# jgsimard/big-dreamer

Hardware: AMD Instinct MI355X
Metric: latent transitions/sec (RSSM + imagination) at batch=50 chunk=50 H=15 (higher is better)
Workload: dtype f32

## Files before the change

### big_dreamer_amd/csrc/bd_device.h

```cpp
#pragma once
#include <hip/hip_runtime.h>
#include <stdint.h>

namespace bd {

typedef float floatx4 __attribute__((ext_vector_type(4)));

#ifndef BD_WAVES
#define BD_WAVES 4
#endif
constexpr int kWaves = BD_WAVES;
constexpr int kThreads = kWaves * 64;
constexpr int kFragFloats = 256;

__device__ __forceinline__ floatx4 mfma16(float a, float b, floatx4 c) {
    return __builtin_amdgcn_mfma_f32_16x16x4f32(a, b, c, 0, 0, 0);
}

__host__ __device__ __forceinline__ int cdiv(int a, int b) { return (a + b - 1) / b; }

__device__ __forceinline__ int bd_tid() {
    int t = threadIdx.x;
    asm volatile("" : "+v"(t));
    return t;
// ... 210 lines not shown

#ifdef BD_STAMPS
#ifndef BD_STAMP_BLOCK
#define BD_STAMP_BLOCK 0
#endif
#ifndef BD_STAMP_THREAD
#define BD_STAMP_THREAD 0
#endif
static __device__ unsigned long long g_dstamps[64];
#define BD_DSTAMP(base, k)                                                                                  \
    do {                                                                                                    \
        if ((base) >= 0 && (base) + (k) < 64 && blockIdx.x == BD_STAMP_BLOCK && threadIdx.x == BD_STAMP_THREAD) \
            g_dstamps[(base) + (k)] = __builtin_amdgcn_s_memtime();                                          \
    } while (0)
#else
#define BD_DSTAMP(base, k)
#endif

__device__ __forceinline__ floatx4 tall_bias(const float* __restrict__ bias, int N, int nb, int lane) {
    const int col0 = nb * 16 + 4 * (lane >> 4);
    floatx4 b = floatx4{0.f, 0.f, 0.f, 0.f};
    if (bias != nullptr && col0 < N) {
        if (col0 + 4 <= N) {
            __builtin_memcpy(&b, bias + col0, 16);
        } else {
#pragma unroll
            for (int r = 0; r < 4; ++r)
                if (col0 + r < N) b[r] = bias[col0 + r];
        }
    }
    return b;
}

template <int NSEG, int RT, int NI, int D, bool TR = false>
__device__ __forceinline__ void linear_sweep(const Seg (&seg)[NSEG], int nb0, floatx4 (*acc)[RT]) {
    const int lane = bd_tid() & 63;
    constexpr bool kSplit = (NI * RT == 1);
    floatx4 acc2 = floatx4{0.f, 0.f, 0.f, 0.f};
#pragma unroll
    for (int s = 0; s < NSEG; ++s) {
        const int Kb = seg[s].Kb;
        const floatx4* __restrict__ X4 = reinterpret_cast<const floatx4*>(seg[s].X) + lane;
        const floatx4* __restrict__ W4 = reinterpret_cast<const floatx4*>(seg[s].W) + lane + (size_t)nb0 * Kb * 64;
        const size_t wstride = (size_t)kWaves * Kb * 64;
        pipelined_k<D>(
            Kb,
            [&](int kb) {
                LinFrag<RT, NI> f;
#pragma unroll
                for (int i = 0; i < NI; ++i) f.b[i] = W4[i * wstride + (size_t)kb * 64];
#pragma unroll
                for (int rt = 0; rt < RT; ++rt) f.a[rt] = X4[(rt * Kb + kb) * 64];
                return f;
            },
            [&](const LinFrag<RT, NI>& f) {
                if constexpr (kSplit) {
                    if constexpr (TR) {
                        acc[0][0] = mfma16(f.b[0][0], f.a[0][0], acc[0][0]);
                        acc2 = mfma16(f.b[0][1], f.a[0][1], acc2);
                        acc[0][0] = mfma16(f.b[0][2], f.a[0][2], acc[0][0]);
                        acc2 = mfma16(f.b[0][3], f.a[0][3], acc2);
                    } else {
                        acc[0][0] = mfma16(f.a[0][0], f.b[0][0], acc[0][0]);
                        acc2 = mfma16(f.a[0][1], f.b[0][1], acc2);
                        acc[0][0] = mfma16(f.a[0][2], f.b[0][2], acc[0][0]);
                        acc2 = mfma16(f.a[0][3], f.b[0][3], acc2);
                    }
                } else {
#pragma unroll
                    for (int j = 0; j < 4; ++j)
#pragma unroll
                        for (int i = 0; i < NI; ++i)
#pragma unroll
                            for (int rt = 0; rt < RT; ++rt)
                                acc[i][rt] = TR ? mfma16(f.b[i][j], f.a[rt][j], acc[i][rt]) : mfma16(f.a[rt][j], f.b[i][j], acc[i][rt]);
                }
            });
    }
    if constexpr (kSplit) acc[0][0] += acc2;
}

template <int NSEG, int RT, int NI, int D, bool TR = false, class Pre, class Epi>
__device__ __forceinline__ void linear_blocks(const Seg (&seg)[NSEG], const float* __restrict__ bias, int N, int nb0,
                                              Pre&& pre, Epi&& epi, int sb = -1) {
    const int lane = bd_tid() & 63;
    BD_DSTAMP(sb, 0);
    decltype(pre(0, 0)) pf[NI][RT];
#pragma unroll
    for (int i = 0; i < NI; ++i)
#pragma unroll
        for (int rt = 0; rt < RT; ++rt) pf[i][rt] = pre(rt, nb0 + i * kWaves);
    floatx4 acc[NI][RT];
#pragma unroll
    for (int i = 0; i < NI; ++i) {
        floatx4 b4;
        if constexpr (TR) {
            b4 = tall_bias(bias, N, nb0 + i * kWaves, lane);
        } else {
            const int col = (nb0 + i * kWaves) * 16 + (lane & 15);
            const float b = (bias != nullptr && col < N) ? bias[col] : 0.f;
            b4 = floatx4{b, b, b, b};
        }
#pragma unroll
        for (int rt = 0; rt < RT; ++rt) acc[i][rt] = b4;
    }
    BD_DSTAMP(sb, 1);
    linear_sweep<NSEG, RT, NI, D, TR>(seg, nb0, acc);
    BD_DSTAMP(sb, 2);
#pragma unroll
    for (int i = 0; i < NI; ++i)
#pragma unroll
        for (int rt = 0; rt < RT; ++rt) epi(rt, nb0 + i * kWaves, acc[i][rt], pf[i][rt]);
    BD_DSTAMP(sb, 3);
}

constexpr int kSplitPairs = 2;
constexpr int kHeadMaxN = 64;
constexpr int kHeadPlainFloats = 2 * 16 * kHeadMaxN;
constexpr int kSplitPartialFloats = kWaves * kSplitPairs * 2 * kFragFloats;
constexpr int kSplitScratchFloats = kSplitPartialFloats + kHeadPlainFloats;

template <int RT, int NSEG, bool TR = false, class Pre, class Epi>
__device__ __forceinline__ void tile_linear_splitk(const Seg (&seg)[NSEG], const float* __restrict__ bias, int N,
                                                   float* __restrict__ scratch, Pre&& pre, Epi&& epi) {
    const int lane = bd_tid() & 63, wave = bd_wave(bd_tid());
    const int Nb = (N + 15) >> 4;
    const int P = Nb * RT;
    const int my_nb = wave / RT, my_rt = wave - my_nb * RT;
    decltype(pre(0, 0)) pf{};
    floatx4 my_bias = floatx4{0.f, 0.f, 0.f, 0.f};
    if (wave < P) {
        pf = pre(my_rt, my_nb);
        if constexpr (TR) {
            my_bias = tall_bias(bias, N, my_nb, lane);
        } else {
            const int col = my_nb * 16 + (lane & 15);
            const float b = (bias != nullptr && col < N) ? bias[col] : 0.f;
            my_bias = floatx4{b, b, b, b};
        }
    }
// ... 16 lines not shown
                    if (kb < Kb && p < P) {
                        const int nb = p / RT, rt = p % RT;
                        xa[i][p] = X4[(rt * Kb + kb) * 64];
                        wb[i][p] = W4[((size_t)nb * Kb + kb) * 64];
                    }
                }
            }
#pragma unroll
            for (int i = 0; i < KW; ++i) {
                const int kb = kb0 + i * kWaves;
#pragma unroll
                for (int p = 0; p < kSplitPairs; ++p) {
                    if (kb < Kb && p < P) {
#pragma unroll
                        for (int j = 0; j < 4; ++j)
                            acc[p] = TR ? mfma16(wb[i][p][j], xa[i][p][j], acc[p]) : mfma16(xa[i][p][j], wb[i][p][j], acc[p]);
                    }
                }
            }
        }
    }
    floatx4* __restrict__ S4 = reinterpret_cast<floatx4*>(scratch);
#pragma unroll
    for (int p = 0; p < kSplitPairs; ++p)
        if (p < P) S4[(wave * kSplitPairs + p) * 64 + lane] = acc[p];
    lds_barrier();
    if (wave < P) {
        floatx4 r = my_bias;
        for (int w = 0; w < kWaves; ++w) r += S4[(w * kSplitPairs + wave) * 64 + lane];
        epi(my_rt, my_nb, r, pf);
    }
}

template <int RT, int NSEG, bool TR = false, class Pre, class Epi>
__device__ __forceinline__ void tile_linear_pre(const Seg (&seg)[NSEG], const float* __restrict__ bias, int N, Pre&& pre,
                                                Epi&& epi, float* __restrict__ scratch = nullptr, int sb = -1) {
    const int wave = bd_wave(bd_tid());
    const int Nb = (N + 15) >> 4;
    if (scratch != nullptr && Nb * RT <= kSplitPairs) {
        tile_linear_splitk<RT, NSEG, TR>(seg, bias, N, scratch, pre, epi);
        return;
    }
#ifndef BD_PIPE_D
#define BD_PIPE_D 2
#endif
    constexpr int D = BD_PIPE_D;
    for (int nb0 = wave; nb0 < Nb; nb0 += 2 * kWaves) {
        if (nb0 + kWaves < Nb) linear_blocks<NSEG, RT, 2, D, TR>(seg, bias, N, nb0, pre, epi, sb);
        else linear_blocks<NSEG, RT, 1, D, TR>(seg, bias, N, nb0, pre, epi, sb);
    }
}

template <int RT, int NSEG, class Epi>
__device__ __forceinline__ void tile_linear_g(const Seg (&seg)[NSEG], const float* __restrict__ bias, int N, Epi&& epi,
                                              float* __restrict__ scratch = nullptr, int sb = -1) {
    tile_linear_pre<RT, NSEG>(seg, bias, N, NoPre{}, [&](int rt, int nb, floatx4 acc, NoPreVal) { epi(rt, nb, acc); },
                              scratch, sb);
}

template <int RT, class Epi>
__device__ __forceinline__ void tile_linear(const float* __restrict__ X, int Kb, const float* __restrict__ Wp,
                                            const float* __restrict__ bias, int N, Epi&& epi,
                                            float* __restrict__ scratch = nullptr) {
    const Seg seg[1] = {{X, Wp, Kb}};
    tile_linear_g<RT, 1>(seg, bias, N, epi, scratch);
}

template <int NSEG, class Epi>
__device__ __forceinline__ void tile_linear_seg(const Seg (&seg)[NSEG], const float* __restrict__ bias, int N,
                                                Epi&& epi, float* __restrict__ scratch = nullptr, int sb = -1) {
    tile_linear_g<1, NSEG>(seg, bias, N, [&](int, int nb, floatx4 acc) { epi(nb, acc); }, scratch, sb);
}
template <int NSEG, class Epi>
__device__ __forceinline__ void tile_linear_seg_tr(const Seg (&seg)[NSEG], const float* __restrict__ bias, int N, Epi&& epi,
                                                   int sb = -1) {
    tile_linear_pre<1, NSEG, true>(seg, bias, N, NoPre{}, [&](int, int nb, floatx4 acc, NoPreVal) { epi(nb, acc); }, nullptr, sb);
}

constexpr int kTallMaxPer = 3;

template <int RT>
struct TallAcc {
    floatx4 main[kTallMaxPer][RT];
    floatx4 left;
};

__host__ __device__ __forceinline__ bool tall_shape_ok(int N, int RT) {
    const int Nb = (N + 15) >> 4, per = Nb / kWaves;
    return per <= kTallMaxPer && (Nb - per * kWaves) * RT <= kWaves;
}

__device__ __forceinline__ bool tall_left_pair(int Nb, int RT, int wave, int& rt, int& nb) {
    const int per = Nb / kWaves, nleft = (Nb - per * kWaves) * RT;
    if (wave >= nleft) return false;
    const int lb = wave / RT;
    rt = wave - lb * RT;
    nb = per * kWaves + lb;
    return true;
}

template <int RT, int NSEG>
__device__ __forceinline__ void tall_sweep(const Seg (&seg)[NSEG], const float* __restrict__ bias, int N, TallAcc<RT>& t) {
    const int lane = bd_tid() & 63, wave = bd_wave(bd_tid());
    const int Nb = (N + 15) >> 4, per = Nb / kWaves;
#pragma unroll
    for (int i = 0; i < kTallMaxPer; ++i) {
        const floatx4 b = i < per ? tall_bias(bias, N, wave + i * kWaves, lane) : floatx4{0.f, 0.f, 0.f, 0.f};
#pragma unroll
        for (int rt = 0; rt < RT; ++rt) t.main[i][rt] = b;
    }
    if (per == 3) linear_sweep<NSEG, RT, 3, 1, true>(seg, wave, t.main);
    else if (per == 2) linear_sweep<NSEG, RT, 2, 1, true>(seg, wave, t.main);
    else if (per == 1) linear_sweep<NSEG, RT, 1, 2, true>(seg, wave, t.main);
    int lrt = 0, lnb = 0;
    if (tall_left_pair(Nb, RT, wave, lrt, lnb)) {
        floatx4 one[1][1] = {{tall_bias(bias, N, lnb, lane)}};
        Seg s1[NSEG];
#pragma unroll
        for (int s = 0; s < NSEG; ++s) s1[s] = Seg{seg[s].X + (size_t)lrt * seg[s].Kb * kFragFloats, seg[s].W, seg[s].Kb};
        linear_sweep<NSEG, 1, 1, 2, true>(s1, lnb, one);
        t.left = one[0][0];
    }
}

template <int RT, class F>
__device__ __forceinline__ void tall_foreach(int N, const TallAcc<RT>& t, F&& f) {
    const int wave = bd_wave(bd_tid());
    const int Nb = (N + 15) >> 4, per = Nb / kWaves;
#pragma unroll
    for (int i = 0; i < kTallMaxPer; ++i)
        if (i < per) {
#pragma unroll
            for (int rt = 0; rt < RT; ++rt) f(rt, wave + i * kWaves, t.main[i][rt]);
        }
    int lrt = 0, lnb = 0;
    if (tall_left_pair(Nb, RT, wave, lrt, lnb)) f(lrt, lnb, t.left);
}

template <int RT, class G>
__device__ __forceinline__ void tall_fill(int N, TallAcc<RT>& t, G&& g) {
    const int wave = bd_wave(bd_tid());
    const int Nb = (N + 15) >> 4, per = Nb / kWaves;
#pragma unroll
    for (int i = 0; i < kTallMaxPer; ++i)
        if (i < per) {
#pragma unroll
// ... 415 lines not shown
```

### big_dreamer_amd/csrc/heads.hip

```cpp
#include "bd_device.h"
#include "bd_host.h"
#include <stdlib.h>

namespace bd {

constexpr int kHeadHidden = BD_HEAD_HIDDEN;

template <int RT, class F>
__device__ __forceinline__ void tall_map(int N, const TallAcc<RT>& t, const TallAcc<RT>& u, TallAcc<RT>& o, F&& f) {
    const int wave = bd_wave(bd_tid());
    const int Nb = (N + 15) >> 4, per = Nb / kWaves;
#pragma unroll
    for (int i = 0; i < kTallMaxPer; ++i)
        if (i < per) {
#pragma unroll
            for (int rt = 0; rt < RT; ++rt) o.main[i][rt] = f(rt, wave + i * kWaves, t.main[i][rt], u.main[i][rt]);
        }
    int lrt = 0, lnb = 0;
    if (tall_left_pair(Nb, RT, wave, lrt, lnb)) o.left = f(lrt, lnb, t.left, u.left);
}

template <int RT>
__device__ __forceinline__ void img_store(float* img, int Nb, int rt, int nb, floatx4 v) {
    *reinterpret_cast<floatx4*>(img + ((rt * Nb + nb) * 64 + (bd_tid() & 63)) * 4) = v;
}

template <int RT, class KA>
__device__ __forceinline__ void head_fwd_bwd(KA ka, int h, const float* xim, float* img, int KbF, int Hd,
                                             int row0, int M, TallAcc<RT>& d0) {
    const auto& H = ka->head[h];
    const int Nb = cdiv(Hd, 16);
    const int lane = bd_tid() & 63, m = lane & 15;
    TallAcc<RT> sv[kHeadHidden];
#pragma unroll
    for (int l = 0; l < kHeadHidden; ++l) {
        const Seg seg[1] = {{l == 0 ? xim : img, H.w[l], l == 0 ? KbF : Nb}};
        TallAcc<RT> t;
        tall_sweep<RT, 1>(seg, H.b[l], Hd, t);
        lds_barrier();
        tall_map<RT>(Hd, t, t, sv[l], [&](int rt, int nb, floatx4 acc, floatx4) {
            floatx4 v;
#pragma unroll
            for (int r = 0; r < 4; ++r) v[r] = elu(acc[r]);
            img_store<RT>(img, Nb, rt, nb, v);
            return v;
        });
        lds_barrier();
    }
    {
        constexpr int kRows = 16 * RT, TPR = kThreads / kRows;
        static_assert(kThreads % kRows == 0 && TPR <= 64 && (TPR & (TPR - 1)) == 0, "threads per row");
        const int tid = bd_tid(), row = tid / TPR, part = tid - row * TPR;
        const int rt = row >> 4, mr = row & 15, n4 = cdiv(Hd, 4);
        const float* base = img + rt * Nb * kFragFloats;
        float s = 0.f;
        for (int c = part; c < n4; c += TPR) {
            const floatx4 v = *reinterpret_cast<const floatx4*>(base + ((c >> 2) * 64 + (c & 3) * 16 + mr) * 4);
#pragma unroll
            for (int r = 0; r < 4; ++r)
                if (4 * c + r < Hd) s += v[r] * H.w_out[4 * c + r];
        }
#pragma unroll
        for (int o = TPR / 2; o > 0; o >>= 1) s += __shfl_xor(s, o, TPR);
        const int grow = row0 + row;
        if (part == 0 && grow < M) H.out[grow] = s + H.b_out[0];
    }
    lds_barrier();
    {
        TallAcc<RT> t;
        tall_map<RT>(Hd, sv[kHeadHidden - 1], sv[kHeadHidden - 1], t, [&](int rt, int nb, floatx4 a, floatx4) {
            const int grow = row0 + rt * 16 + m;
            const float d = grow < M ? H.dout[grow] : 0.f;
            const floatx4 w = tall_bias(H.w_out, Hd, nb, lane);
            floatx4 v;
#pragma unroll
            for (int r = 0; r < 4; ++r) v[r] = d * w[r] * elu_grad_from_out(a[r]);
            img_store<RT>(img, Nb, rt, nb, v);
            return v;
        });
        lds_barrier();
    }
#pragma unroll
    for (int l = kHeadHidden - 1; l >= 1; --l) {
        const Seg seg[1] = {{img, H.wt[l], Nb}};
        TallAcc<RT> t;
        tall_sweep<RT, 1>(seg, nullptr, Hd, t);
        if (l > 1) lds_barrier();
        tall_map<RT>(Hd, t, sv[l - 1], l > 1 ? t : d0, [&](int rt, int nb, floatx4 acc, floatx4 a) {
            const bool in = row0 + rt * 16 + m < M;
            const int col0 = nb * 16 + 4 * (lane >> 4);
            floatx4 v = floatx4{0.f, 0.f, 0.f, 0.f};
#pragma unroll
            for (int r = 0; r < 4; ++r)
                if (in && col0 + r < Hd) v[r] = acc[r] * elu_grad_from_out(a[r]);
            if (l > 1) img_store<RT>(img, Nb, rt, nb, v);
            return v;
        });
        if (l > 1) lds_barrier();
    }
}

template <int RT>
__global__ __launch_bounds__(kThreads) __attribute__((amdgpu_waves_per_eu(4 - RT, 4 - RT))) void img_heads_kernel(bd_img_heads_args a) {
    extern __shared__ __attribute__((aligned(16))) float smem[];
    const int KbF = cdiv(a.F, 16), Nb = cdiv(a.Hd, 16);
    float* xim = smem;
    float* img = smem + (size_t)RT * (KbF > Nb ? KbF : Nb) * kFragFloats;
    const int row0 = blockIdx.x * 16 * RT;
    if (tile_pairs_ok(a.x, a.F, a.F, nullptr, 0))
        load_tile_concat_pairs<RT>(xim, KbF, row0, a.M, a.x, a.F, a.F, nullptr, 0, 0);
    else
        load_tile_concat<RT>(xim, KbF, row0, a.M, a.x, a.F, a.F, nullptr, 0, 0);
    lds_barrier();
    BD_KARGS(bd_img_heads_args, ka);
    TallAcc<RT> d0r, d0v;
#pragma unroll 1
    for (int h = 0; h < 2; ++h) {
        BD_KARGS_FRESH(ka);
        TallAcc<RT> d0;
        head_fwd_bwd<RT>(ka, h, xim, img, KbF, a.Hd, row0, a.M, d0);
        if (h == 0) d0r = d0;
        else d0v = d0;
    }
    lds_barrier();
    tall_foreach2<RT>(a.Hd, d0r, d0v, [&](int rt, int nb, floatx4 r, floatx4 v) {
        img_store<RT>(xim, Nb, rt, nb, r);
        img_store<RT>(img, Nb, rt, nb, v);
    });
    lds_barrier();
    const Seg segs[2] = {{xim, a.head[0].wt[0], Nb}, {img, a.head[1].wt[0], Nb}};
    const bool rows_full = row0 + 16 * RT <= a.M;
    tile_linear_g<RT, 2>(segs, nullptr, a.F, [&](int rt, int nb, floatx4 acc) {
        const int ln = bd_tid() & 63, col = nb * 16 + (ln & 15);
        const unsigned r0 = (unsigned)(row0 + rt * 16 + 4 * (ln >> 4));
        if (col >= a.F) return;
        float* __restrict__ p = a.dx + (r0 * (unsigned)a.F + (unsigned)col);
#pragma unroll
        for (int r = 0; r < 4; ++r)
            if (rows_full || (int)r0 + r < a.M) p[r * (unsigned)a.F] = acc[r];
    });
}

static int heads_rt(int Hd) {
    static const char* force = getenv("BD_HEADS_RT");
    const bool two = !(force && atoi(force) == 1) && tall_shape_ok(Hd, 2);
    return two ? 2 : (tall_shape_ok(Hd, 1) ? 1 : 0);
}

static size_t heads_lds(int RT, int F, int Hd) {
    const int KbF = cdiv(F, 16), Nb = cdiv(Hd, 16);
    return (size_t)RT * ((KbF > Nb ? KbF : Nb) + Nb) * kFragFloats * sizeof(float);
}

}

extern "C" {

int bd_img_heads_supported(int F, int Hd) {
    using namespace bd;
    if (F <= 0 || Hd <= 0) return 0;
    const int rt = heads_rt(Hd);
    return rt > 0 && heads_lds(rt, F, Hd) <= (size_t)kMaxLds;
}

int bd_img_heads_fwd_bwd(const bd_img_heads_args* a, void* stream) {
    using namespace bd;
    BD_REQUIRE(a && a->M > 0 && a->x && a->dx, "bd_img_heads_fwd_bwd: bad M / x / dx");
    BD_REQUIRE(bd_img_heads_supported(a->F, a->Hd), "bd_img_heads_fwd_bwd: F=%d, Hd=%d not covered (Hd <= 240 in "
               "column blocks the waves can balance, LDS <= %d B)", a->F, a->Hd, kMaxLds);
    BD_REQUIRE((size_t)a->M * (size_t)a->F < ((size_t)1 << 31), "bd_img_heads_fwd_bwd: M*F=%zu needs 64-bit offsets",
               (size_t)a->M * (size_t)a->F);
    for (int h = 0; h < 2; ++h) {
        const bd_img_head& H = a->head[h];
        bool ok = H.w_out && H.b_out && H.dout && H.out;
        for (int l = 0; l < BD_HEAD_HIDDEN; ++l) ok = ok && H.w[l] && H.wt[l] && H.b[l];
        BD_REQUIRE(ok, "bd_img_heads_fwd_bwd: head %d is missing an operand", h);
    }
    const int rt = heads_rt(a->Hd);
    const size_t lds = heads_lds(rt, a->F, a->Hd);
    const dim3 grid(cdiv(a->M, 16 * rt));
    if (rt == 2) {
        if (lds > 64 * 1024 && allow_big_lds(img_heads_kernel<2>)) return -1;
        hipLaunchKernelGGL(img_heads_kernel<2>, grid, dim3(kThreads), lds, (hipStream_t)stream, *a);
    } else {
        if (lds > 64 * 1024 && allow_big_lds(img_heads_kernel<1>)) return -1;
        hipLaunchKernelGGL(img_heads_kernel<1>, grid, dim3(kThreads), lds, (hipStream_t)stream, *a);
    }
    BD_CHECK_LAUNCH("bd_img_heads_fwd_bwd");
    return 0;
}

}
```

### big_dreamer_amd/_cabi.py

```python
from __future__ import annotations

import ctypes as C
import os

import torch

_HERE = os.path.dirname(os.path.abspath(__file__))
LIB_PATH = os.environ.get("BD_LIB") or os.path.join(_HERE, "libbigdreamer_hip.so")

if not os.path.exists(LIB_PATH):
    raise ImportError(
        f"{LIB_PATH} is missing: the MI355X HIP extension has not been built "
        "(run `python -c 'import __graft_entry__ as g; g.build()'`). There is no CPU fallback.")

lib = C.CDLL(LIB_PATH)

BD_MAX_LAYERS = 6
ACT_NONE, ACT_ELU, ACT_ELU_GRAD = 0, 1, 2
P = C.c_void_p
F32 = C.c_float
I32 = C.c_int


class PackDesc(C.Structure):
# ... 165 lines not shown
    "bd_observe_backward_cluster": (I32, [C.POINTER(ObserveBwdArgs), P, C.c_size_t, P]),
    "bd_observe_cluster_status": (I32, [P, I32, P]),
    "bd_observe_cluster_err_offset": (C.c_size_t, [I32]),
    "bd_observe_cluster_set_spin_limit": (I32, [C.c_uint]),
    "bd_observe_cluster_set_ksplit": (I32, [I32]),
    "bd_gauss_head_forward": (I32, [P, P, I32, I32, F32, P, P, P, P]),
    "bd_gauss_head_backward": (I32, [P, P, P, P, P, I32, I32, P, P]),
    "bd_observe_cat_forward": (I32, [C.POINTER(ObserveCatFwdArgs), P]),
    "bd_observe_cat_backward": (I32, [C.POINTER(ObserveCatBwdArgs), P]),
    "bd_observe_cat_cluster_size": (I32, [I32, I32, I32, I32, I32]),
    "bd_observe_cat_cluster_ws_floats": (C.c_size_t, [I32, I32, I32, I32, I32]),
    "bd_observe_cat_forward_cluster": (I32, [C.POINTER(ObserveCatFwdArgs), I32, P, C.c_size_t, P]),
    "bd_observe_cat_backward_cluster": (I32, [C.POINTER(ObserveCatBwdArgs), I32, P, C.c_size_t, P]),
    "bd_imagine_cat_forward": (I32, [C.POINTER(ImagineCatFwdArgs), P]),
    "bd_imagine_cat_backward": (I32, [C.POINTER(ImagineCatBwdArgs), P]),
    "bd_imagine_forward": (I32, [C.POINTER(ImagineFwdArgs), P]),
    "bd_imagine_forward_scan": (I32, [C.POINTER(ImagineFwdArgs), P]),
    "bd_actor_entropy": (I32, [P, P, P, I32, I32, I32, I32, P]),
    "bd_imagine_backward": (I32, [C.POINTER(ImagineBwdArgs), P]),
    "bd_lambda_return_forward": (I32, [P, P, I32, I32, F32, F32, P, P]),
    "bd_rng_fill": (I32, [C.POINTER(RngFillArgs), P]),
    "bd_philox4x32_10": (I32, [C.POINTER(C.c_uint), C.POINTER(C.c_uint), C.POINTER(C.c_uint)]),
    "bd_actor_entropy_rng": (I32, [C.c_ulonglong, C.c_ulonglong, C.c_uint, P, P, I32, I32, I32, I32, P]),
    "bd_gemm_nt": (I32, [P, I32, P, I32, P, I32, I32, I32, I32, I32, P]),
    "bd_categorical_head_forward": (I32, [P, P, I32, I32, I32, P, P, P]),
    "bd_categorical_head_backward": (I32, [P, P, I32, I32, I32, P, P]),
    "bd_kl_categorical_forward": (I32, [P, P, I32, I32, I32, F32, I32, P, I32, P, P]),
    "bd_kl_categorical_backward": (I32, [P, P, I32, I32, I32, F32, F32, F32, F32, P, I32, P, P, P]),
    "bd_plan_rollout": (I32, [C.POINTER(PlanArgs), P]),
    "bd_cem_refit": (I32, [P, I32, P, I32, I32, I32, I32, I32, P, P, P]),
    "bd_lambda_return_backward": (I32, [P, F32, I32, I32, F32, F32, P, P, P]),
    "bd_img_heads_supported": (I32, [I32, I32]),
    "bd_img_heads_fwd_bwd": (I32, [C.POINTER(ImgHeadsArgs), P]),
    "bd_actor_reinforce": (I32, [P, P, P, P, P, P, P, I32, I32, I32, F32, F32, F32, I32, P, P, I32, P, P]),
    "bd_actor_reinforce_cat": (I32, [P, P, P, P, P, P, I32, I32, I32, F32, F32, F32, I32, P, P, I32, P, P]),
    "bd_normal_nll": (I32, [P, I32, P, I32, I32, I32, F32, P, I32, P, I32, P, P]),
    "bd_bernoulli_nll": (I32, [P, P, C.c_size_t, F32, P, P, I32, P, P]),
    "bd_kl_forward": (I32, [P, P, P, P, I32, I32, F32, I32, P, I32, P, P]),
    "bd_kl_backward": (I32, [P, P, P, P, I32, I32, F32, F32, F32, F32, P, I32, P, P, P, P, P]),
    "bd_sum": (I32, [P, C.c_size_t, P, I32, P, P]),
    "bd_sumsq": (I32, [P, C.c_size_t, P, I32, P, P]),
    "bd_adam_step": (I32, [P, P, P, P, C.c_size_t, F32, F32, F32, F32, F32, I32, F32, P, I32, P]),
    "bd_polyak": (I32, [P, P, C.c_size_t, F32, P]),
    "bd_replay_gather": (I32, [P, P, I32, I32, P, P]),
    "bd_replay_gather_pixels": (I32, [P, P, I32, I32, I32, P, P, P]),
    "bd_replay_gather_pixels_rng": (I32, [P, P, I32, I32, I32, C.c_ulonglong, C.c_ulonglong, P, P]),
    "bd_reduce_ws_floats": (C.c_size_t, []),
    "bd_conv_gemm": (I32, [C.POINTER(ConvArgs), P]),
    "bd_conv_thin_forward": (I32, [P, I32, I32, I32, I32, I32, P, I32, P, I32, P, P, P]),
    "bd_conv_pack_class": (I32, [P, P, I32, I32, I32, I32, I32, I32, I32, P]),
    "bd_conv_pack_fused": (I32, [P, P, I32, I32, I32, P]),
    "bd_elu_backward": (I32, [P, P, C.c_size_t, P]),
    "bd_image_layout": (I32, [P, P, I32, I32, I32, I32, P]),
    "bd_colsum_ws_floats": (C.c_size_t, [I32]),
    "bd_colsum": (I32, [P, C.c_size_t, I32, P, P, P]),
}

for _name, (_res, _args) in _SIGS.items():
    _fn = getattr(lib, _name)
    _fn.restype = _res
    _fn.argtypes = _args

EXPORTED = tuple(_SIGS)


def check(rc: int) -> None:
# ... 22 lines not shown
```

### include/bigdreamer_hip.h

```cpp
#ifndef BIGDREAMER_HIP_H
#define BIGDREAMER_HIP_H

#include <stddef.h>
#include <stdint.h>

#ifdef __cplusplus
extern "C" {
#endif

#define BD_MAX_LAYERS 6
#define BD_ACT_NONE 0
#define BD_ACT_ELU 1
#define BD_ACT_ELU_GRAD 2

const char* bd_last_error(void);
int bd_version(void);

typedef struct {
    const float* src;
    float* dst;
    int ld;
    int N, K;
    int transpose;
} bd_pack_desc;
// ... 196 lines not shown
    float min_std;
    const float* dfeat;
    float dentropy;
    float* d_actor_pre;
    float* d_actor_out;
    const float* ent_weight;
    int discrete_actions;
} bd_imagine_bwd_args;
int bd_imagine_backward(const bd_imagine_bwd_args* a, void* stream);

int bd_lambda_return_forward(const float* reward, const float* value, int Hm, int N, float discount,
                             float lambda_, float* returns, void* stream);
int bd_lambda_return_backward(const float* dreturns, float dret_const, int Hm, int N, float discount,
                              float lambda_, float* dreward, float* dvalue, void* stream);

#define BD_HEAD_HIDDEN 4
typedef struct {
    const float* w[BD_HEAD_HIDDEN];
    const float* wt[BD_HEAD_HIDDEN];
    const float* b[BD_HEAD_HIDDEN];
    const float* w_out;
    const float* b_out;
    const float* dout;
    float* out;
} bd_img_head;
typedef struct {
    int M, F, Hd;
    const float* x;
    bd_img_head head[2];
    float* dx;
} bd_img_heads_args;
int bd_img_heads_supported(int F, int Hd);
int bd_img_heads_fwd_bwd(const bd_img_heads_args* a, void* stream);

int bd_actor_reinforce(const float* eps_action, const float* act_us, const float* act_stats, const float* returns,
                       const float* base0, const float* value, const float* weight, int Hm, int N, int A, float rho,
                       float grad_scale, float dentropy, int write, float* d_actor_out, float* scalars, int slot, float* ws,
                       void* stream);
int bd_actor_reinforce_cat(const float* action, const float* act_stats, const float* returns, const float* base0,
                           const float* value, const float* weight, int Hm, int N, int A, float rho, float grad_scale,
                           float dentropy, int write, float* d_actor_out, float* scalars, int slot, float* ws,
                           void* stream);

#define BD_RNG_MAX_TENSORS 6
#define BD_RNG_NORMAL 0
#define BD_RNG_EXPONENTIAL 1
typedef struct {
    int n;
    unsigned long long seed;
    unsigned long long step;
    struct {
        float* p;
        size_t count;
        int kind;
        unsigned stream_id;
    } t[BD_RNG_MAX_TENSORS];
} bd_rng_fill_args;
int bd_rng_fill(const bd_rng_fill_args* a, void* stream);
int bd_philox4x32_10(const unsigned* ctr4, const unsigned* key2, unsigned* out4);
int bd_actor_entropy_rng(unsigned long long seed, unsigned long long step, unsigned stream_id, float* act_stats,
                         float* entropy, int Hm, int N, int A, int n_samples, void* stream);

int bd_gemm_nt(const float* A, int lda, const float* B, int ldb, float* C, int ldc, int M, int N, int K, int accumulate,
               void* stream);

int bd_categorical_head_forward(const float* logits, const float* q_noise, int rows, int D, int C, float* state,
// ... 156 lines not shown
```

Measured before the change: 13.28 million.

## Balance img heads grid by splitting leftover rows into single-tile tail blocks

The image heads kernel now plans its grid from the device's resident block slots. It runs full 32-row tiles in whole waves of slots and covers the leftover 16-row units with RT=1 tail blocks, instead of a ragged last wave of 32-row blocks. Tail blocks use a OneChain variant that drops the split dual accumulator chain in the single-block MFMA sweep. This aims to cut the wave-quantization imbalance at the end of the grid, at the cost of an occupancy query, extra template instantiations and lower per-block efficiency for the tail tiles.

```diff
diff --git a/big_dreamer_amd/csrc/bd_device.h b/big_dreamer_amd/csrc/bd_device.h
--- a/big_dreamer_amd/csrc/bd_device.h
+++ b/big_dreamer_amd/csrc/bd_device.h
@@ -266,10 +266,10 @@
     return b;
 }
 
-template <int NSEG, int RT, int NI, int D, bool TR = false>
+template <int NSEG, int RT, int NI, int D, bool TR = false, bool OneChain = false>
 __device__ __forceinline__ void linear_sweep(const Seg (&seg)[NSEG], int nb0, floatx4 (*acc)[RT]) {
     const int lane = bd_tid() & 63;
-    constexpr bool kSplit = (NI * RT == 1);
+    constexpr bool kSplit = (NI * RT == 1) && !OneChain;
     floatx4 acc2 = floatx4{0.f, 0.f, 0.f, 0.f};
 #pragma unroll
     for (int s = 0; s < NSEG; ++s) {
@@ -314,7 +314,7 @@
     if constexpr (kSplit) acc[0][0] += acc2;
 }
 
-template <int NSEG, int RT, int NI, int D, bool TR = false, class Pre, class Epi>
+template <int NSEG, int RT, int NI, int D, bool TR = false, bool OneChain = false, class Pre, class Epi>
 __device__ __forceinline__ void linear_blocks(const Seg (&seg)[NSEG], const float* __restrict__ bias, int N, int nb0,
                                               Pre&& pre, Epi&& epi, int sb = -1) {
     const int lane = bd_tid() & 63;
@@ -339,7 +339,7 @@
         for (int rt = 0; rt < RT; ++rt) acc[i][rt] = b4;
     }
     BD_DSTAMP(sb, 1);
-    linear_sweep<NSEG, RT, NI, D, TR>(seg, nb0, acc);
+    linear_sweep<NSEG, RT, NI, D, TR, OneChain>(seg, nb0, acc);
     BD_DSTAMP(sb, 2);
 #pragma unroll
     for (int i = 0; i < NI; ++i)
@@ -422,7 +422,7 @@
     }
 }
 
-template <int RT, int NSEG, bool TR = false, class Pre, class Epi>
+template <int RT, int NSEG, bool TR = false, bool OneChain = false, class Pre, class Epi>
 __device__ __forceinline__ void tile_linear_pre(const Seg (&seg)[NSEG], const float* __restrict__ bias, int N, Pre&& pre,
                                                 Epi&& epi, float* __restrict__ scratch = nullptr, int sb = -1) {
     const int wave = bd_wave(bd_tid());
@@ -436,16 +436,16 @@
 #endif
     constexpr int D = BD_PIPE_D;
     for (int nb0 = wave; nb0 < Nb; nb0 += 2 * kWaves) {
-        if (nb0 + kWaves < Nb) linear_blocks<NSEG, RT, 2, D, TR>(seg, bias, N, nb0, pre, epi, sb);
-        else linear_blocks<NSEG, RT, 1, D, TR>(seg, bias, N, nb0, pre, epi, sb);
-    }
-}
-
-template <int RT, int NSEG, class Epi>
+        if (nb0 + kWaves < Nb) linear_blocks<NSEG, RT, 2, D, TR, OneChain>(seg, bias, N, nb0, pre, epi, sb);
+        else linear_blocks<NSEG, RT, 1, D, TR, OneChain>(seg, bias, N, nb0, pre, epi, sb);
+    }
+}
+
+template <int RT, int NSEG, bool OneChain = false, class Epi>
 __device__ __forceinline__ void tile_linear_g(const Seg (&seg)[NSEG], const float* __restrict__ bias, int N, Epi&& epi,
                                               float* __restrict__ scratch = nullptr, int sb = -1) {
-    tile_linear_pre<RT, NSEG>(seg, bias, N, NoPre{}, [&](int rt, int nb, floatx4 acc, NoPreVal) { epi(rt, nb, acc); },
-                              scratch, sb);
+    tile_linear_pre<RT, NSEG, false, OneChain>(
+        seg, bias, N, NoPre{}, [&](int rt, int nb, floatx4 acc, NoPreVal) { epi(rt, nb, acc); }, scratch, sb);
 }
 
 template <int RT, class Epi>
@@ -489,7 +489,7 @@
     return true;
 }
 
-template <int RT, int NSEG>
+template <int RT, int NSEG, bool OneChain = false>
 __device__ __forceinline__ void tall_sweep(const Seg (&seg)[NSEG], const float* __restrict__ bias, int N, TallAcc<RT>& t) {
     const int lane = bd_tid() & 63, wave = bd_wave(bd_tid());
     const int Nb = (N + 15) >> 4, per = Nb / kWaves;
@@ -501,7 +501,7 @@
     }
     if (per == 3) linear_sweep<NSEG, RT, 3, 1, true>(seg, wave, t.main);
     else if (per == 2) linear_sweep<NSEG, RT, 2, 1, true>(seg, wave, t.main);
-    else if (per == 1) linear_sweep<NSEG, RT, 1, 2, true>(seg, wave, t.main);
+    else if (per == 1) linear_sweep<NSEG, RT, 1, 2, true, OneChain>(seg, wave, t.main);
     int lrt = 0, lnb = 0;
     if (tall_left_pair(Nb, RT, wave, lrt, lnb)) {
         floatx4 one[1][1] = {{tall_bias(bias, N, lnb, lane)}};
diff --git a/big_dreamer_amd/csrc/heads.hip b/big_dreamer_amd/csrc/heads.hip
--- a/big_dreamer_amd/csrc/heads.hip
+++ b/big_dreamer_amd/csrc/heads.hip
@@ -25,7 +25,7 @@
     *reinterpret_cast<floatx4*>(img + ((rt * Nb + nb) * 64 + (bd_tid() & 63)) * 4) = v;
 }
 
-template <int RT, class KA>
+template <int RT, int kOutRows, bool OneChain, class KA>
 __device__ __forceinline__ void head_fwd_bwd(KA ka, int h, const float* xim, float* img, int KbF, int Hd,
                                              int row0, int M, TallAcc<RT>& d0) {
     const auto& H = ka->head[h];
@@ -36,7 +36,7 @@
     for (int l = 0; l < kHeadHidden; ++l) {
         const Seg seg[1] = {{l == 0 ? xim : img, H.w[l], l == 0 ? KbF : Nb}};
         TallAcc<RT> t;
-        tall_sweep<RT, 1>(seg, H.b[l], Hd, t);
+        tall_sweep<RT, 1, OneChain>(seg, H.b[l], Hd, t);
         lds_barrier();
         tall_map<RT>(Hd, t, t, sv[l], [&](int rt, int nb, floatx4 acc, floatx4) {
             floatx4 v;
@@ -48,10 +48,11 @@
         lds_barrier();
     }
     {
-        constexpr int kRows = 16 * RT, TPR = kThreads / kRows;
-        static_assert(kThreads % kRows == 0 && TPR <= 64 && (TPR & (TPR - 1)) == 0, "threads per row");
+        constexpr int TPR = kThreads / kOutRows;
+        static_assert(kOutRows >= 16 * RT && kThreads % kOutRows == 0 && TPR <= 64 && (TPR & (TPR - 1)) == 0,
+                      "threads per row");
         const int tid = bd_tid(), row = tid / TPR, part = tid - row * TPR;
-        const int rt = row >> 4, mr = row & 15, n4 = cdiv(Hd, 4);
+        const int rt = row >> 4, mr = row & 15, n4 = row < 16 * RT ? cdiv(Hd, 4) : 0;
         const float* base = img + rt * Nb * kFragFloats;
         float s = 0.f;
         for (int c = part; c < n4; c += TPR) {
@@ -63,7 +64,7 @@
 #pragma unroll
         for (int o = TPR / 2; o > 0; o >>= 1) s += __shfl_xor(s, o, TPR);
         const int grow = row0 + row;
-        if (part == 0 && grow < M) H.out[grow] = s + H.b_out[0];
+        if (part == 0 && row < 16 * RT && grow < M) H.out[grow] = s + H.b_out[0];
     }
     lds_barrier();
     {
@@ -84,7 +85,7 @@
     for (int l = kHeadHidden - 1; l >= 1; --l) {
         const Seg seg[1] = {{img, H.wt[l], Nb}};
         TallAcc<RT> t;
-        tall_sweep<RT, 1>(seg, nullptr, Hd, t);
+        tall_sweep<RT, 1, OneChain>(seg, nullptr, Hd, t);
         if (l > 1) lds_barrier();
         tall_map<RT>(Hd, t, sv[l - 1], l > 1 ? t : d0, [&](int rt, int nb, floatx4 acc, floatx4 a) {
             const bool in = row0 + rt * 16 + m < M;
@@ -100,13 +101,11 @@
     }
 }
 
-template <int RT>
-__global__ __launch_bounds__(kThreads) __attribute__((amdgpu_waves_per_eu(4 - RT, 4 - RT))) void img_heads_kernel(bd_img_heads_args a) {
-    extern __shared__ __attribute__((aligned(16))) float smem[];
+template <int RT, int kOutRows, bool OneChain>
+__device__ __forceinline__ void img_heads_tile(const bd_img_heads_args& a, int row0, float* smem) {
     const int KbF = cdiv(a.F, 16), Nb = cdiv(a.Hd, 16);
     float* xim = smem;
     float* img = smem + (size_t)RT * (KbF > Nb ? KbF : Nb) * kFragFloats;
-    const int row0 = blockIdx.x * 16 * RT;
     if (tile_pairs_ok(a.x, a.F, a.F, nullptr, 0))
         load_tile_concat_pairs<RT>(xim, KbF, row0, a.M, a.x, a.F, a.F, nullptr, 0, 0);
     else
@@ -118,7 +117,7 @@
     for (int h = 0; h < 2; ++h) {
         BD_KARGS_FRESH(ka);
         TallAcc<RT> d0;
-        head_fwd_bwd<RT>(ka, h, xim, img, KbF, a.Hd, row0, a.M, d0);
+        head_fwd_bwd<RT, kOutRows, OneChain>(ka, h, xim, img, KbF, a.Hd, row0, a.M, d0);
         if (h == 0) d0r = d0;
         else d0v = d0;
     }
@@ -130,7 +129,7 @@
     lds_barrier();
     const Seg segs[2] = {{xim, a.head[0].wt[0], Nb}, {img, a.head[1].wt[0], Nb}};
     const bool rows_full = row0 + 16 * RT <= a.M;
-    tile_linear_g<RT, 2>(segs, nullptr, a.F, [&](int rt, int nb, floatx4 acc) {
+    tile_linear_g<RT, 2, OneChain>(segs, nullptr, a.F, [&](int rt, int nb, floatx4 acc) {
         const int ln = bd_tid() & 63, col = nb * 16 + (ln & 15);
         const unsigned r0 = (unsigned)(row0 + rt * 16 + 4 * (ln >> 4));
         if (col >= a.F) return;
@@ -141,6 +140,20 @@
     });
 }
 
+template <int RT>
+__global__ __launch_bounds__(kThreads) __attribute__((amdgpu_waves_per_eu(4 - RT, 4 - RT))) void img_heads_kernel(
+    bd_img_heads_args a, int n_main) {
+    extern __shared__ __attribute__((aligned(16))) float smem[];
+    const int b = blockIdx.x;
+    if constexpr (RT == 2) {
+        if (b >= n_main) {
+            img_heads_tile<1, 32, true>(a, n_main * 32 + (b - n_main) * 16, smem);
+            return;
+        }
+    }
+    img_heads_tile<RT, 16 * RT, false>(a, b * 16 * RT, smem);
+}
+
 static int heads_rt(int Hd) {
     static const char* force = getenv("BD_HEADS_RT");
     const bool two = !(force && atoi(force) == 1) && tall_shape_ok(Hd, 2);
@@ -150,6 +163,31 @@
 static size_t heads_lds(int RT, int F, int Hd) {
     const int KbF = cdiv(F, 16), Nb = cdiv(Hd, 16);
     return (size_t)RT * ((KbF > Nb ? KbF : Nb) + Nb) * kFragFloats * sizeof(float);
+}
+
+static int heads_slots(size_t lds) {
+    thread_local int dev_c = -1, slots_c = 0;
+    thread_local size_t lds_c = 0;
+    int dev = 0;
+    if (hipGetDevice(&dev) != hipSuccess) return 0;
+    if (dev != dev_c || lds != lds_c) {
+        int cus = 0, per_cu = 0;
+        if (hipDeviceGetAttribute(&cus, hipDeviceAttributeMultiprocessorCount, dev) != hipSuccess ||
+            hipOccupancyMaxActiveBlocksPerMultiprocessor(&per_cu, img_heads_kernel<2>, kThreads, lds) != hipSuccess)
+            return 0;
+        dev_c = dev, lds_c = lds, slots_c = cus * per_cu;
+    }
+    return slots_c;
+}
+
+static void heads_plan(int M, int slots, int& n_main, int& n_tail) {
+    const char* e = getenv("BD_HEADS_PLAN");
+    const int units = cdiv(M, 16);
+    n_main = cdiv(units, 2), n_tail = 0;
+    if ((e && atoi(e) == 0) || slots <= 0) return;
+    const int full = units / (2 * slots) * slots;
+    const int rest = units - 2 * full;
+    if (rest <= slots) n_main = full, n_tail = rest;
 }
 
 }
@@ -178,13 +216,16 @@
     }
     const int rt = heads_rt(a->Hd);
     const size_t lds = heads_lds(rt, a->F, a->Hd);
-    const dim3 grid(cdiv(a->M, 16 * rt));
     if (rt == 2) {
         if (lds > 64 * 1024 && allow_big_lds(img_heads_kernel<2>)) return -1;
-        hipLaunchKernelGGL(img_heads_kernel<2>, grid, dim3(kThreads), lds, (hipStream_t)stream, *a);
+        int n_main = 0, n_tail = 0;
+        heads_plan(a->M, heads_slots(lds), n_main, n_tail);
+        hipLaunchKernelGGL(img_heads_kernel<2>, dim3(n_main + n_tail), dim3(kThreads), lds, (hipStream_t)stream, *a,
+                           n_main);
     } else {
         if (lds > 64 * 1024 && allow_big_lds(img_heads_kernel<1>)) return -1;
-        hipLaunchKernelGGL(img_heads_kernel<1>, grid, dim3(kThreads), lds, (hipStream_t)stream, *a);
+        const int n = cdiv(a->M, 16);
+        hipLaunchKernelGGL(img_heads_kernel<1>, dim3(n), dim3(kThreads), lds, (hipStream_t)stream, *a, n);
     }
     BD_CHECK_LAUNCH("bd_img_heads_fwd_bwd");
     return 0;
```

Measured after the change: 13.34 million, median of 6. No clear change (+0.4%).

## Balance imagination heads grid by mixing 32-row and 16-row tiles to fill wave

Applied to the files above, without the earlier changes.

The imagination heads kernel gets a planned launch. Most row tiles stay 32 rows, and the tail that would spill into a partial extra wave of blocks is split into 16-row tiles, sized from the device's CU count and occupancy. The 16-row tiles reuse the RT=2 launch configuration with half the rows active and turn off the split-accumulator MFMA path. The goal is to shrink the tail-wave imbalance at the end of the grid. The cost is an occupancy query (cached per device and shape) and idle threads in the 16-row blocks.

```diff
diff --git a/big_dreamer_amd/_cabi.py b/big_dreamer_amd/_cabi.py
--- a/big_dreamer_amd/_cabi.py
+++ b/big_dreamer_amd/_cabi.py
@@ -221,6 +221,8 @@
     "bd_lambda_return_backward": (I32, [P, F32, I32, I32, F32, F32, P, P, P]),
     "bd_img_heads_supported": (I32, [I32, I32]),
     "bd_img_heads_fwd_bwd": (I32, [C.POINTER(ImgHeadsArgs), P]),
+    "bd_img_heads_fwd_bwd_mode": (I32, [C.POINTER(ImgHeadsArgs), I32, P]),
+    "bd_img_heads_plan": (I32, [I32, I32, C.POINTER(I32), C.POINTER(I32)]),
     "bd_actor_reinforce": (I32, [P, P, P, P, P, P, P, I32, I32, I32, F32, F32, F32, I32, P, P, I32, P, P]),
     "bd_actor_reinforce_cat": (I32, [P, P, P, P, P, P, I32, I32, I32, F32, F32, F32, I32, P, P, I32, P, P]),
     "bd_normal_nll": (I32, [P, I32, P, I32, I32, I32, F32, P, I32, P, I32, P, P]),
diff --git a/big_dreamer_amd/csrc/bd_device.h b/big_dreamer_amd/csrc/bd_device.h
--- a/big_dreamer_amd/csrc/bd_device.h
+++ b/big_dreamer_amd/csrc/bd_device.h
@@ -266,10 +266,10 @@
     return b;
 }
 
-template <int NSEG, int RT, int NI, int D, bool TR = false>
+template <int NSEG, int RT, int NI, int D, bool TR = false, bool SPLIT = true>
 __device__ __forceinline__ void linear_sweep(const Seg (&seg)[NSEG], int nb0, floatx4 (*acc)[RT]) {
     const int lane = bd_tid() & 63;
-    constexpr bool kSplit = (NI * RT == 1);
+    constexpr bool kSplit = SPLIT && (NI * RT == 1);
     floatx4 acc2 = floatx4{0.f, 0.f, 0.f, 0.f};
 #pragma unroll
     for (int s = 0; s < NSEG; ++s) {
@@ -314,7 +314,7 @@
     if constexpr (kSplit) acc[0][0] += acc2;
 }
 
-template <int NSEG, int RT, int NI, int D, bool TR = false, class Pre, class Epi>
+template <int NSEG, int RT, int NI, int D, bool TR = false, bool SPLIT = true, class Pre, class Epi>
 __device__ __forceinline__ void linear_blocks(const Seg (&seg)[NSEG], const float* __restrict__ bias, int N, int nb0,
                                               Pre&& pre, Epi&& epi, int sb = -1) {
     const int lane = bd_tid() & 63;
@@ -339,7 +339,7 @@
         for (int rt = 0; rt < RT; ++rt) acc[i][rt] = b4;
     }
     BD_DSTAMP(sb, 1);
-    linear_sweep<NSEG, RT, NI, D, TR>(seg, nb0, acc);
+    linear_sweep<NSEG, RT, NI, D, TR, SPLIT>(seg, nb0, acc);
     BD_DSTAMP(sb, 2);
 #pragma unroll
     for (int i = 0; i < NI; ++i)
@@ -422,7 +422,7 @@
     }
 }
 
-template <int RT, int NSEG, bool TR = false, class Pre, class Epi>
+template <int RT, int NSEG, bool TR = false, bool SPLIT = true, class Pre, class Epi>
 __device__ __forceinline__ void tile_linear_pre(const Seg (&seg)[NSEG], const float* __restrict__ bias, int N, Pre&& pre,
                                                 Epi&& epi, float* __restrict__ scratch = nullptr, int sb = -1) {
     const int wave = bd_wave(bd_tid());
@@ -436,15 +436,15 @@
 #endif
     constexpr int D = BD_PIPE_D;
     for (int nb0 = wave; nb0 < Nb; nb0 += 2 * kWaves) {
-        if (nb0 + kWaves < Nb) linear_blocks<NSEG, RT, 2, D, TR>(seg, bias, N, nb0, pre, epi, sb);
-        else linear_blocks<NSEG, RT, 1, D, TR>(seg, bias, N, nb0, pre, epi, sb);
-    }
-}
-
-template <int RT, int NSEG, class Epi>
+        if (nb0 + kWaves < Nb) linear_blocks<NSEG, RT, 2, D, TR, SPLIT>(seg, bias, N, nb0, pre, epi, sb);
+        else linear_blocks<NSEG, RT, 1, D, TR, SPLIT>(seg, bias, N, nb0, pre, epi, sb);
+    }
+}
+
+template <int RT, int NSEG, bool SPLIT = true, class Epi>
 __device__ __forceinline__ void tile_linear_g(const Seg (&seg)[NSEG], const float* __restrict__ bias, int N, Epi&& epi,
                                               float* __restrict__ scratch = nullptr, int sb = -1) {
-    tile_linear_pre<RT, NSEG>(seg, bias, N, NoPre{}, [&](int rt, int nb, floatx4 acc, NoPreVal) { epi(rt, nb, acc); },
+    tile_linear_pre<RT, NSEG, false, SPLIT>(seg, bias, N, NoPre{}, [&](int rt, int nb, floatx4 acc, NoPreVal) { epi(rt, nb, acc); },
                               scratch, sb);
 }
 
@@ -489,7 +489,7 @@
     return true;
 }
 
-template <int RT, int NSEG>
+template <int RT, int NSEG, bool SPLIT = true>
 __device__ __forceinline__ void tall_sweep(const Seg (&seg)[NSEG], const float* __restrict__ bias, int N, TallAcc<RT>& t) {
     const int lane = bd_tid() & 63, wave = bd_wave(bd_tid());
     const int Nb = (N + 15) >> 4, per = Nb / kWaves;
@@ -501,7 +501,7 @@
     }
     if (per == 3) linear_sweep<NSEG, RT, 3, 1, true>(seg, wave, t.main);
     else if (per == 2) linear_sweep<NSEG, RT, 2, 1, true>(seg, wave, t.main);
-    else if (per == 1) linear_sweep<NSEG, RT, 1, 2, true>(seg, wave, t.main);
+    else if (per == 1) linear_sweep<NSEG, RT, 1, 2, true, SPLIT>(seg, wave, t.main);
     int lrt = 0, lnb = 0;
     if (tall_left_pair(Nb, RT, wave, lrt, lnb)) {
         floatx4 one[1][1] = {{tall_bias(bias, N, lnb, lane)}};
diff --git a/big_dreamer_amd/csrc/heads.hip b/big_dreamer_amd/csrc/heads.hip
--- a/big_dreamer_amd/csrc/heads.hip
+++ b/big_dreamer_amd/csrc/heads.hip
@@ -1,5 +1,6 @@
 #include "bd_device.h"
 #include "bd_host.h"
+#include <mutex>
 #include <stdlib.h>
 
 namespace bd {
@@ -25,7 +26,7 @@
     *reinterpret_cast<floatx4*>(img + ((rt * Nb + nb) * 64 + (bd_tid() & 63)) * 4) = v;
 }
 
-template <int RT, class KA>
+template <int RT, bool MATCH, class KA>
 __device__ __forceinline__ void head_fwd_bwd(KA ka, int h, const float* xim, float* img, int KbF, int Hd,
                                              int row0, int M, TallAcc<RT>& d0) {
     const auto& H = ka->head[h];
@@ -36,7 +37,7 @@
     for (int l = 0; l < kHeadHidden; ++l) {
         const Seg seg[1] = {{l == 0 ? xim : img, H.w[l], l == 0 ? KbF : Nb}};
         TallAcc<RT> t;
-        tall_sweep<RT, 1>(seg, H.b[l], Hd, t);
+        tall_sweep<RT, 1, !MATCH>(seg, H.b[l], Hd, t);
         lds_barrier();
         tall_map<RT>(Hd, t, t, sv[l], [&](int rt, int nb, floatx4 acc, floatx4) {
             floatx4 v;
@@ -48,22 +49,25 @@
         lds_barrier();
     }
     {
-        constexpr int kRows = 16 * RT, TPR = kThreads / kRows;
+        static_assert(!MATCH || RT == 1, "MATCH is the 16-row form of the 32-row tile");
+        constexpr int kRows = 16 * RT, TPR = kThreads / (MATCH ? 32 : kRows);
         static_assert(kThreads % kRows == 0 && TPR <= 64 && (TPR & (TPR - 1)) == 0, "threads per row");
         const int tid = bd_tid(), row = tid / TPR, part = tid - row * TPR;
-        const int rt = row >> 4, mr = row & 15, n4 = cdiv(Hd, 4);
-        const float* base = img + rt * Nb * kFragFloats;
-        float s = 0.f;
-        for (int c = part; c < n4; c += TPR) {
-            const floatx4 v = *reinterpret_cast<const floatx4*>(base + ((c >> 2) * 64 + (c & 3) * 16 + mr) * 4);
-#pragma unroll
-            for (int r = 0; r < 4; ++r)
-                if (4 * c + r < Hd) s += v[r] * H.w_out[4 * c + r];
+        if (!MATCH || row < kRows) {
+            const int rt = row >> 4, mr = row & 15, n4 = cdiv(Hd, 4);
+            const float* base = img + rt * Nb * kFragFloats;
+            float s = 0.f;
+            for (int c = part; c < n4; c += TPR) {
+                const floatx4 v = *reinterpret_cast<const floatx4*>(base + ((c >> 2) * 64 + (c & 3) * 16 + mr) * 4);
+#pragma unroll
+                for (int r = 0; r < 4; ++r)
+                    if (4 * c + r < Hd) s += v[r] * H.w_out[4 * c + r];
+            }
+#pragma unroll
+            for (int o = TPR / 2; o > 0; o >>= 1) s += __shfl_xor(s, o, TPR);
+            const int grow = row0 + row;
+            if (part == 0 && grow < M) H.out[grow] = s + H.b_out[0];
         }
-#pragma unroll
-        for (int o = TPR / 2; o > 0; o >>= 1) s += __shfl_xor(s, o, TPR);
-        const int grow = row0 + row;
-        if (part == 0 && grow < M) H.out[grow] = s + H.b_out[0];
     }
     lds_barrier();
     {
@@ -84,7 +88,7 @@
     for (int l = kHeadHidden - 1; l >= 1; --l) {
         const Seg seg[1] = {{img, H.wt[l], Nb}};
         TallAcc<RT> t;
-        tall_sweep<RT, 1>(seg, nullptr, Hd, t);
+        tall_sweep<RT, 1, !MATCH>(seg, nullptr, Hd, t);
         if (l > 1) lds_barrier();
         tall_map<RT>(Hd, t, sv[l - 1], l > 1 ? t : d0, [&](int rt, int nb, floatx4 acc, floatx4 a) {
             const bool in = row0 + rt * 16 + m < M;
@@ -100,13 +104,11 @@
     }
 }
 
-template <int RT>
-__global__ __launch_bounds__(kThreads) __attribute__((amdgpu_waves_per_eu(4 - RT, 4 - RT))) void img_heads_kernel(bd_img_heads_args a) {
-    extern __shared__ __attribute__((aligned(16))) float smem[];
+template <int RT, bool MATCH>
+__device__ __forceinline__ void heads_tile(const bd_img_heads_args& a, int row0, float* smem) {
     const int KbF = cdiv(a.F, 16), Nb = cdiv(a.Hd, 16);
     float* xim = smem;
     float* img = smem + (size_t)RT * (KbF > Nb ? KbF : Nb) * kFragFloats;
-    const int row0 = blockIdx.x * 16 * RT;
     if (tile_pairs_ok(a.x, a.F, a.F, nullptr, 0))
         load_tile_concat_pairs<RT>(xim, KbF, row0, a.M, a.x, a.F, a.F, nullptr, 0, 0);
     else
@@ -118,7 +120,7 @@
     for (int h = 0; h < 2; ++h) {
         BD_KARGS_FRESH(ka);
         TallAcc<RT> d0;
-        head_fwd_bwd<RT>(ka, h, xim, img, KbF, a.Hd, row0, a.M, d0);
+        head_fwd_bwd<RT, MATCH>(ka, h, xim, img, KbF, a.Hd, row0, a.M, d0);
         if (h == 0) d0r = d0;
         else d0v = d0;
     }
@@ -130,7 +132,7 @@
     lds_barrier();
     const Seg segs[2] = {{xim, a.head[0].wt[0], Nb}, {img, a.head[1].wt[0], Nb}};
     const bool rows_full = row0 + 16 * RT <= a.M;
-    tile_linear_g<RT, 2>(segs, nullptr, a.F, [&](int rt, int nb, floatx4 acc) {
+    tile_linear_g<RT, 2, !MATCH>(segs, nullptr, a.F, [&](int rt, int nb, floatx4 acc) {
         const int ln = bd_tid() & 63, col = nb * 16 + (ln & 15);
         const unsigned r0 = (unsigned)(row0 + rt * 16 + 4 * (ln >> 4));
         if (col >= a.F) return;
@@ -141,6 +143,19 @@
     });
 }
 
+template <int RT>
+__global__ __launch_bounds__(kThreads) __attribute__((amdgpu_waves_per_eu(4 - RT, 4 - RT))) void img_heads_kernel(bd_img_heads_args a) {
+    extern __shared__ __attribute__((aligned(16))) float smem[];
+    heads_tile<RT, false>(a, blockIdx.x * 16 * RT, smem);
+}
+
+__global__ __launch_bounds__(kThreads) __attribute__((amdgpu_waves_per_eu(2, 2))) void img_heads_plan_kernel(bd_img_heads_args a, int n32) {
+    extern __shared__ __attribute__((aligned(16))) float smem[];
+    const int b = blockIdx.x;
+    if (b < n32) heads_tile<2, false>(a, b * 32, smem);
+    else heads_tile<1, true>(a, n32 * 32 + (b - n32) * 16, smem);
+}
+
 static int heads_rt(int Hd) {
     static const char* force = getenv("BD_HEADS_RT");
     const bool two = !(force && atoi(force) == 1) && tall_shape_ok(Hd, 2);
@@ -150,6 +165,32 @@
 static size_t heads_lds(int RT, int F, int Hd) {
     const int KbF = cdiv(F, 16), Nb = cdiv(Hd, 16);
     return (size_t)RT * ((KbF > Nb ? KbF : Nb) + Nb) * kFragFloats * sizeof(float);
+}
+
+static void heads_plan(int M, int slots, int& n32, int& n16) {
+    const int t32 = cdiv(M, 32);
+    const int full = slots > 0 ? t32 / slots * slots : t32;
+    n32 = t32, n16 = 0;
+    if (full < t32 && cdiv(M - 32 * full, 16) <= slots) n32 = full, n16 = cdiv(M - 32 * full, 16);
+}
+
+static int heads_slots(int F, int Hd, size_t lds) {
+    struct Entry { int dev, F, Hd, slots; };
+    static Entry cache[8];
+    static int n = 0;
+    static std::mutex mu;
+    int dev = 0;
+    if (hipGetDevice(&dev) != hipSuccess) return 0;
+    std::lock_guard<std::mutex> lock(mu);
+    for (int i = 0; i < n; ++i)
+        if (cache[i].dev == dev && cache[i].F == F && cache[i].Hd == Hd) return cache[i].slots;
+    int cus = 0, per_cu = 0;
+    if (hipDeviceGetAttribute(&cus, hipDeviceAttributeMultiprocessorCount, dev) != hipSuccess ||
+        hipOccupancyMaxActiveBlocksPerMultiprocessor(&per_cu, img_heads_plan_kernel, kThreads, lds) != hipSuccess)
+        cus = per_cu = 0, (void)hipGetLastError();
+    const int slots = cus * per_cu;
+    if (n < 8) cache[n++] = Entry{dev, F, Hd, slots};
+    return slots;
 }
 
 }
@@ -163,7 +204,13 @@
     return rt > 0 && heads_lds(rt, F, Hd) <= (size_t)kMaxLds;
 }
 
-int bd_img_heads_fwd_bwd(const bd_img_heads_args* a, void* stream) {
+int bd_img_heads_plan(int M, int slots, int* n32, int* n16) {
+    if (M <= 0 || !n32 || !n16) return -1;
+    bd::heads_plan(M, slots, *n32, *n16);
+    return 0;
+}
+
+int bd_img_heads_fwd_bwd_mode(const bd_img_heads_args* a, int plan, void* stream) {
     using namespace bd;
     BD_REQUIRE(a && a->M > 0 && a->x && a->dx, "bd_img_heads_fwd_bwd: bad M / x / dx");
     BD_REQUIRE(bd_img_heads_supported(a->F, a->Hd), "bd_img_heads_fwd_bwd: F=%d, Hd=%d not covered (Hd <= 240 in "
@@ -176,8 +223,22 @@
         for (int l = 0; l < BD_HEAD_HIDDEN; ++l) ok = ok && H.w[l] && H.wt[l] && H.b[l];
         BD_REQUIRE(ok, "bd_img_heads_fwd_bwd: head %d is missing an operand", h);
     }
+    if (plan < 0) {
+        static const char* env = getenv("BD_HEADS_PLAN");
+        plan = !(env && atoi(env) == 0);
+    }
     const int rt = heads_rt(a->Hd);
     const size_t lds = heads_lds(rt, a->F, a->Hd);
+    if (rt == 2 && plan) {
+        if (lds > 64 * 1024 && allow_big_lds(img_heads_plan_kernel)) return -1;
+        int n32 = 0, n16 = 0;
+        heads_plan(a->M, heads_slots(a->F, a->Hd, lds), n32, n16);
+        if (n16 > 0) {
+            hipLaunchKernelGGL(img_heads_plan_kernel, dim3(n32 + n16), dim3(kThreads), lds, (hipStream_t)stream, *a, n32);
+            BD_CHECK_LAUNCH("bd_img_heads_fwd_bwd");
+            return 0;
+        }
+    }
     const dim3 grid(cdiv(a->M, 16 * rt));
     if (rt == 2) {
         if (lds > 64 * 1024 && allow_big_lds(img_heads_kernel<2>)) return -1;
@@ -190,4 +251,8 @@
     return 0;
 }
 
-}
+int bd_img_heads_fwd_bwd(const bd_img_heads_args* a, void* stream) {
+    return bd_img_heads_fwd_bwd_mode(a, -1, stream);
+}
+
+}
diff --git a/include/bigdreamer_hip.h b/include/bigdreamer_hip.h
--- a/include/bigdreamer_hip.h
+++ b/include/bigdreamer_hip.h
@@ -252,6 +252,8 @@
 } bd_img_heads_args;
 int bd_img_heads_supported(int F, int Hd);
 int bd_img_heads_fwd_bwd(const bd_img_heads_args* a, void* stream);
+int bd_img_heads_fwd_bwd_mode(const bd_img_heads_args* a, int plan, void* stream);
+int bd_img_heads_plan(int M, int slots, int* n32, int* n16);
 
 int bd_actor_reinforce(const float* eps_action, const float* act_us, const float* act_stats, const float* returns,
                        const float* base0, const float* value, const float* weight, int Hm, int N, int A, float rho,
```

After: 13.20 million before, 13.26 million after, median of 6. Within noise of the previous version (+0.5%).
